# IBM/mcp-context-forge

Hardware: AMD Instinct MI355X
Metric: tool_call_req_per_s (higher is better)
Workload: dtype bf16

## Files before the change

### mcp_context_forge_amd/gpu/classifier.py

```python

from __future__ import annotations

import torch

from ..models.classifier import HashedTextClassifier
from ..ops import hip


class GpuClassifier:
    def __init__(self, model: HashedTextClassifier, device: str = "cuda"):
        self.dim = model.dim
        self.hidden = model.hidden
        self.classes = model.classes
        assert self.dim % 64 == 0 and self.hidden % 128 == 0, "MFMA tile constraints"
        with torch.no_grad():
            self.w1t = model.w1.t().contiguous().to(device=device, dtype=torch.bfloat16)
            self.b1 = model.b1.to(device=device, dtype=torch.float32).contiguous()
            self.w2t = model.w2.t().contiguous().to(device=device, dtype=torch.bfloat16)
            self.b2 = model.b2.to(device=device, dtype=torch.float32).contiguous()

    def forward(self, feats_bf16: torch.Tensor) -> torch.Tensor:
        h = hip.gemm_bt(feats_bf16, self.w1t, self.b1, act=hip.ACT_GELU, out_bf16=True)
        return hip.gemv_head(h, self.w2t, self.b2, act=hip.ACT_SIGMOID)

    def forward_into(self, feats_bf16: torch.Tensor, h_buf: torch.Tensor,
                     scores_buf: torch.Tensor) -> None:
        hip.gemm_bt(feats_bf16, self.w1t, self.b1, act=hip.ACT_GELU, out_bf16=True, out=h_buf)
        hip.gemv_head(h_buf, self.w2t, self.b2, act=hip.ACT_SIGMOID, out=scores_buf)
```

### mcp_context_forge_amd/gpu/pipeline.py

```python

from __future__ import annotations

import asyncio
import json
import time
from typing import Any, Dict, List, Optional, Tuple

import numpy as np
import torch

from ..ops import dfa, hip
from ..ops.entropy import TOL as ENTROPY_TOL
from ..protocol import jsonrpc
from ..plugins.builtin import _walk_strings
from ..plugins.framework import PluginMode
from .batch import pack_texts, pad_rows
from .classifier import GpuClassifier
from .semcache import GpuSemanticCache, tool_hash

_NORMALIZE_TRIGGERS = ["\\t", "\\n", "\\r", "\\f", "\\u", "  ", '" ', ' "',
                       "[" + chr(0x80) + "-" + chr(0xFF) + "]"]

_SCHEMA_NEST_PATTERNS = [":\\{", ":\\["]

_TYPED_PAT = {
    "string": '"{k}":"',
    "number": '"{k}":[0-9\\-]',
    "integer": '"{k}":[0-9\\-]',
    "boolean": '"{k}":[tf]',
    "array": '"{k}":\\[',
}


class _ToolMeta:
    __slots__ = ("tool", "name", "tid", "itype", "thash", "native_kind", "native_client",
                 "client", "handler", "schema_mode", "required_bits", "typed_pairs",
                 "has_output_schema", "original_name", "reachable", "host_chain", "a2a_fast")

    def __init__(self):
        self.schema_mode = "host"
        self.required_bits = 0
        self.typed_pairs: List[Tuple[int, int]] = []
        self.native_kind = -1
        self.native_client = None
        self.client = None
        self.handler = None
        self.has_output_schema = False
        self.host_chain = False
        self.a2a_fast = False


class _PackedRows:

    __slots__ = ("blob", "offs")

    def __init__(self, blob: bytes, offs: np.ndarray):
        self.blob = blob
        self.offs = offs

    def __len__(self) -> int:
        return max(int(self.offs.shape[0]) - 1, 0)

    def __getitem__(self, i: int) -> bytes:
        return self.blob[int(self.offs[i]):int(self.offs[i + 1])]


class _IndexedUsers:

    __slots__ = ("users", "uidx")

    def __init__(self, users: List[Optional[str]], uidx: np.ndarray):
# ... 126 lines not shown

        self.banks["postmeta"] = hip.DeviceScanTables(
            dfa.compile_literals(['"structuredContent"'], case_insensitive=False), device)

        self._bankset3 = hip.ScanBankSet(
            [(n, self.banks[n]) for n in ("pii", "regex", "harm", "postmeta", "secrets")
             if n in self.banks],
            device)
        self._bankset1: Optional[hip.ScanBankSet] = None
        self._graphs = None
        self._graphs3 = None

        self._slot_store = hip.store_new(self.semcache.capacity) if self.semcache is not None else 0
        self._exact_native = hip.cache_new(self.exact_cache.ttl) if self.exact_cache is not None else 0

        def _strtable(items):
            blob = b"".join(x.encode() for x in items)
            off = np.zeros(len(items) + 1, dtype=np.int32)
            for i, x in enumerate(items):
                off[i + 1] = off[i] + len(x.encode())
            return np.frombuffer(blob, dtype=np.uint8).copy() if blob else np.zeros(1, dtype=np.uint8), off

        from ..models.classifier import category_names

        self._deny_tab = _strtable(self.deny.words if self.deny else [])
        self._harm_tab = _strtable(self.harm.cats if self.harm else [])
        self._mod_tab = _strtable(category_names(self.moderation.model.classes) if self.moderation else [])

        self._meta_gen = -1
        self._plugins_ver = -1
        self._toolmap = 0
        self._meta_list: List[_ToolMeta] = []
        self._tool_meta: Dict[str, _ToolMeta] = {}
        self._schema_bank: Optional[hip.DeviceScanTables] = None
        self._schema_pat_ids: Dict[str, int] = {}
        self._nest_bits = 0

        self.batches = 0
        self.requests = 0
        self.fast_path = 0
        self.slow_path = 0
        self.blocked = 0
        self.cache_hits = 0
        self.post_rewrites = 0
        self.post_c = 0
        self.post_c_punt = 0
        self.py_fallback = 0
        self.host_bound = 0
        self.secrets_routed = 0
        import os as _os

        self.timing_enabled = bool(_os.environ.get("FORGE_PIPELINE_TIMING"))
        self.timing: Dict[str, float] = {}

    def _schema_pattern(self, pat: str) -> int:
        pid = self._schema_pat_ids.get(pat)
        if pid is None:
            pid = len(self._schema_pat_ids)
            self._schema_pat_ids[pat] = pid
        return pid

    def _esc_key(self, k: str) -> Optional[str]:
        if not k or not all(c.isalnum() or c == "_" for c in k):
            return None
        return k

    def _compile_tool_schema(self, meta: _ToolMeta, schema: Optional[dict]) -> None:
        if self.schema_guard is None or not schema:
            meta.schema_mode = "trivial"
            return
        if not (schema.get("properties") or schema.get("required") or
                schema.get("additionalProperties") is False or schema.get("anyOf") or
                schema.get("allOf") or schema.get("oneOf")):
            meta.schema_mode = "trivial"
            return
        props = schema.get("properties") or {}
        required = schema.get("required") or []
        if schema.get("additionalProperties") is False or schema.get("anyOf") or \
           schema.get("allOf") or schema.get("oneOf"):
            meta.schema_mode = "host"
            return
        req_bits = 0
        pairs: List[Tuple[int, int]] = []
        for k, sub in props.items():
            ek = self._esc_key(k)
            ty = sub.get("type") if isinstance(sub, dict) else None
            extra = isinstance(sub, dict) and any(
                c in sub for c in ("enum", "const", "pattern", "minimum", "maximum", "minLength",
                                   "maxLength", "minItems", "maxItems", "properties", "items",
                                   "anyOf", "allOf", "oneOf", "exclusiveMinimum", "exclusiveMaximum"))
            if ek is None or extra or (ty is not None and not isinstance(ty, str)) or \
               (ty is not None and ty not in _TYPED_PAT and ty not in ("object", "null")):
                meta.schema_mode = "host"
                return
            present = self._schema_pattern(f'"{ek}":')
            if ty in _TYPED_PAT:
                typed = self._schema_pattern(_TYPED_PAT[ty].format(k=ek))
                pairs.append((present, typed))
            if k in required:
                req_bits |= 1 << present
        for k in required:
            if k not in props:
                ek = self._esc_key(k)
                if ek is None:
                    meta.schema_mode = "host"
                    return
# ... 863 lines not shown
                    else:
                        punted.append(j)
                nat_set = set(nat_idx)
                py_js = [j for j in rewrite_js if j not in nat_set] + punted
                py_js.sort()
        self._toc("rw_c", t_sub)
        t_sub = self._tic()

        for j in py_js:
            mt = self._meta_list[tool_idx[j]]
            r = int(rows[j])
            idb = self._id_bytes(blob, env, r)
            try:
                args = json.loads(blob[args_b[j]:args_e[j]].tobytes() or b"{}")
            except Exception:
                responses[r] = self._splice_error(idb, jsonrpc.INVALID_PARAMS, "invalid arguments")
                continue
            if self.deny is not None and self._t_rw_deny[tool_idx[j]]:
                hay = _text_of(args)
                hay = hay.lower() if self.deny.case_insensitive else hay
                word = next((w for w in self.deny.words
                             if (w.lower() if self.deny.case_insensitive else w) in hay), None)
                if word is not None:
                    responses[r] = self._splice_error(
                        idb, jsonrpc.POLICY_DENIED, f"deny_filter: deny word {word!r} present")
                    self.blocked += 1
                    continue
            status, payload = self._apply_rewrites(
                mt.name, args,
                do_norm=bool(norm_m[j]) if norm_m is not None else True,
                do_regex=bool(regex_m[j]) if regex_m is not None else True,
                do_pii=bool(pii_m[j]) if pii_m is not None else True,
                pii_bits=int(pii_m[j]) if pii_m is not None else -1)
            if status == "__block__":
                responses[r] = self._splice_error(idb, jsonrpc.POLICY_DENIED, payload)
                self.blocked += 1
                continue
            if self.harm is not None and self._t_rw_harm[tool_idx[j]]:
                hay2 = _text_of(payload).lower()
                for w, ph in enumerate(self.harm.phrases):
                    if ph.lower() in hay2:
                        harm_c[j] = w
                        break
            ok_items.append((j, payload))
        self._toc("rw_pyloop", t_sub)
        if not ok_items:
            return None
        t_sub = self._tic()

        texts2 = [scan_bytes[j] if j in scan_bytes
                  else json.dumps(a, separators=(",", ":"), sort_keys=True, default=str).encode()
                  for (j, a) in ok_items]
        scores2_t = None
        if self.classifier is not None:
            data2, beg2, end2 = pack_texts(texts2, self.device)
            f2, _ = hip.featurize(data2, beg2, end2, self.feat_dim, pad_to=128)
            scores2_t = self.classifier.forward(f2)[: len(ok_items)]

        self._toc("rw_launch", t_sub)
        async def finish() -> List[Tuple[int, Any]]:
            return await self._finish_rewrite(ok_items, harm_c, schema_c, scores2_t,
                                              blob, env, rows, tool_idx, hit, hit_slot, responses)

        return finish

    async def _finish_rewrite(self, ok_items, harm_c, schema_c, scores2_t,
                              blob, env, rows, tool_idx, hit, hit_slot,
                              responses: List[Optional[bytes]]) -> List[Tuple[int, Any]]:
        t_sub = self._tic()
        if scores2_t is not None:
            await self._await_gpu()
        self._toc("rw_sync", t_sub)
        t_sub = self._tic()
        scores2 = scores2_t.cpu().numpy() if scores2_t is not None else None

        mod_on = scores2 is not None and self._enforcing(self.moderation)
        sc_max = scores2.max(axis=1) if mod_on else None
        sc_arg = scores2.argmax(axis=1) if mod_on else None
        mod_thr = self.moderation.threshold if mod_on else 0.0
        sg_on = self._enforcing(self.schema_guard)
        if mod_on:
            from ..models.classifier import category_names
            cat_names = category_names(scores2.shape[1])
        if sg_on:
            from ..utils.jsonschema import validate as _validate
        mod_app, harm_cats = self._t_mod_app, (self.harm.cats if self.harm else [])

        out: List[Tuple[int, Any]] = []
        for jj, (j, args2) in enumerate(ok_items):
            ti = tool_idx[j]
            if mod_on and mod_app[ti] and float(sc_max[jj]) >= mod_thr:
                r = int(rows[j])
                cat = cat_names[int(sc_arg[jj])]
                responses[r] = self._splice_error(
                    self._id_bytes(blob, env, r), jsonrpc.POLICY_DENIED,
                    f"content_moderation: moderation: category {cat} score {float(sc_max[jj]):.3f}")
                self.blocked += 1
                continue
            hj = harm_c.get(j, -1)
            if hj >= 0:
                r = int(rows[j])
                cat = harm_cats[hj] if hj < len(harm_cats) else "?"
                responses[r] = self._splice_error(
                    self._id_bytes(blob, env, r), jsonrpc.POLICY_DENIED,
                    f"harmful_content_detector: harmful content ({cat})")
                self.blocked += 1
                continue
            if sg_on and schema_c.get(j, 2) == 1:
                pass
            elif sg_on and self._meta_list[ti].schema_mode != "trivial":
                mt = self._meta_list[ti]
                if isinstance(args2, bytes):
                    args2 = json.loads(args2)
                errs = _validate(args2 or {}, mt.tool.get("input_schema") or {})
                if errs:
                    r = int(rows[j])
                    responses[r] = self._splice_error(
                        self._id_bytes(blob, env, r), jsonrpc.POLICY_DENIED,
                        "schema_guard: schema violation: " + "; ".join(errs[:5]))
                    self.blocked += 1
                    continue
            if hit[j]:
                r = int(rows[j])
                res = self._cache_result_bytes(int(hit_slot[j]))
                idb = self._id_bytes(blob, env, r)
                if idb is not None and res is not None:
                    responses[r] = self._splice_result(idb, res)
# ... 373 lines not shown

            new = _walk_strings(result, fn)
            if found and self.pii.action == "block" and self._enforcing(self.pii):
                return rb, True, f"pii_filter: PII detected: {sorted(set(found))}"
            if found and self.pii.action == "mask":
                result = new
        if mt.has_output_schema and isinstance(result, dict):
            from ..utils.jsonschema import validate as _validate

            payload = result.get("structuredContent", result)
            errs = _validate(payload, mt.tool.get("output_schema") or {})
            if errs:
                result = {"content": [{"type": "text", "text": "output schema violation: " + "; ".join(errs[:3])}],
                          "isError": True}
        if self.harm is not None and self._enforcing(self.harm) and self._applies(self.harm, name):
            hay = json.dumps(result, separators=(",", ":"), sort_keys=True, default=str).lower()
            for phrase, cat in zip(self.harm.phrases, self.harm.cats):
                if phrase.lower() in hay:
                    return rb, True, f"harmful_content_detector: harmful content ({cat})"
        if self.toon is not None and self._applies(self.toon, name) and isinstance(result, dict):
            new = self.toon.encode_result(result)
            if new is not None:
                result = new
        if self.out_guard is not None and isinstance(result, dict):
            total = sum(len(c.get("text", "")) for c in result.get("content", []) if isinstance(c, dict))
            if total > self.out_guard.max_chars and self.out_guard.action == "truncate":
                result = dict(result)
                result["content"] = [
                    {**c, "text": c["text"][: self.out_guard.max_chars]}
                    if isinstance(c, dict) and isinstance(c.get("text"), str) else c
                    for c in result.get("content", [])
                ]
        is_err = bool(isinstance(result, dict) and result.get("isError"))
        return json.dumps(result, separators=(",", ":"), default=str).encode(), is_err, None

    def _breaker_record(self, name: str, is_error: bool) -> None:
        b = self.breaker
        st = b._st(name)
        st["results"].append(is_error)
        if len(st["results"]) > b.window:
            st["results"] = st["results"][-b.window:]
        if len(st["results"]) >= b.window and (sum(st["results"]) / len(st["results"])) >= b.error_threshold:
            st["open_until"] = time.monotonic() + b.cooldown
            st["results"] = []

    def stats(self) -> Dict[str, Any]:
        out = {
            "timing_s": {k: round(v, 4) for k, v in self.timing.items()} if self.timing_enabled else None,
            "batches": self.batches, "requests": self.requests, "fast_path": self.fast_path,
            "slow_path": self.slow_path, "blocked": self.blocked, "cache_hits": self.cache_hits,
            "host_bound": self.host_bound, "secrets_routed": self.secrets_routed,
            "post_rewrites": self.post_rewrites, "post_c": self.post_c,
            "post_c_punt": self.post_c_punt, "py_fallback": self.py_fallback,
            "banks": {k: {"states": v.n_states, "classes": v.n_classes} for k, v in self.banks.items()},
        }
        if self.semcache is not None:
            out["semcache"] = self.semcache.stats()
        return out
```

### mcp_context_forge_amd/ops/build.py

```python

from __future__ import annotations

import os
import subprocess
import sys
from pathlib import Path

CSRC = Path(__file__).parent / "csrc"
LIB = Path(__file__).parent / "libforge_hip.so"
ARCH = os.environ.get("PYTORCH_ROCM_ARCH", "gfx950")
HIPCC = os.environ.get("HIPCC", "/opt/rocm/bin/hipcc")

SOURCES = ["scan.hip", "entropy.hip", "featurize.hip", "json_guard.hip", "gemm_bf16.hip", "runtime.hip",
           "gemm_v2.hip", "envelope.cpp", "upstream.cpp", "fastpath.cpp", "rewrite.cpp", "pool.cpp"]


PYBRIDGE = Path(__file__).parent / "forge_pybridge.so"
EDGE = Path(__file__).parent / "forge_edge.so"
HEY = Path(__file__).parent / "forge_hey"


def needs_build() -> bool:
    if not LIB.exists():
        return True
    lib_mtime = LIB.stat().st_mtime
    watched = [CSRC / f for f in SOURCES] + sorted(CSRC.glob("*.h"))
    return any(f.stat().st_mtime > lib_mtime for f in watched)


def build_pybridge(force: bool = False, verbose: bool = True) -> Path:
    src = CSRC / "pybridge.c"
    if not force and PYBRIDGE.exists() and PYBRIDGE.stat().st_mtime > src.stat().st_mtime:
        return PYBRIDGE
    import sysconfig

    cc = os.environ.get("CC", "gcc")
    cmd = [cc, "-O2", "-fPIC", "-shared", f"-I{sysconfig.get_paths()['include']}",
           "-o", str(PYBRIDGE), str(src)]
    if verbose:
        print("[forge-pybridge]", " ".join(cmd), file=sys.stderr)
    subprocess.run(cmd, check=True)
    return PYBRIDGE


def build_edge(force: bool = False, verbose: bool = True) -> Path:
    src = CSRC / "edge.cpp"
    newest = max(src.stat().st_mtime, (CSRC / "edge_pack.hpp").stat().st_mtime)
    if not force and EDGE.exists() and EDGE.stat().st_mtime > newest:
        return EDGE
    import sysconfig

    cxx = os.environ.get("CXX", "g++")
    cmd = [cxx, "-O2", "-std=c++17", "-fPIC", "-shared", "-pthread",
           f"-I{sysconfig.get_paths()['include']}", "-o", str(EDGE), str(src)]
    if verbose:
        print("[forge-edge]", " ".join(cmd), file=sys.stderr)
    subprocess.run(cmd, check=True)
    return EDGE


def build_hey(force: bool = False, verbose: bool = True) -> Path:
    src = CSRC / "forge_hey.cpp"
    if not force and HEY.exists() and HEY.stat().st_mtime > src.stat().st_mtime:
        return HEY
    cxx = os.environ.get("CXX", "g++")
    cmd = [cxx, "-O2", "-std=c++17", "-pthread", "-o", str(HEY), str(src)]
    if verbose:
# ... 31 lines not shown
```

### mcp_context_forge_amd/ops/csrc/forge_api.h

```cpp
#ifndef FORGE_API_H
#define FORGE_API_H

#include <stdint.h>

#define FORGE_ACT_NONE 0
#define FORGE_ACT_GELU 1
#define FORGE_ACT_SIGMOID 2

#define FORGE_ERR_SHAPE 9001
#define FORGE_ERR_ACT 9002
#define FORGE_ERR_GEMV_K 9003
#define FORGE_ERR_ROW_ALIGN 9004

#define FORGE_SCAN_LDS_LIMIT (64 * 1024)
#define FORGE_SCAN_TABLE_BYTES(n_states, n_classes) \
    ((int64_t)(n_states) * (n_classes) * 2 + 256 + (int64_t)(n_states) * 4)

typedef void (*forge_task_fn)(int index, void* ctx);

#ifdef __cplusplus
extern "C" {
#endif


// ... 74 lines not shown

int64_t forge_decide(
    const uint8_t* blob, const int32_t* id_beg, const int32_t* id_end,
    const int32_t* args_beg, const int32_t* args_end, const int32_t* tool_idx,
    const int32_t* name_beg, const int32_t* name_end,
    const uint32_t* deny_m, const uint32_t* harm_m, const uint32_t* pii_m,
    const uint32_t* regex_m, const uint32_t* norm_m, const uint32_t* schema_m,
    const uint8_t* mod_block, const int32_t* mod_cat, const float* mod_score,
    const uint8_t* hit, const int32_t* hit_slot, const uint64_t* user_hash, int m,
    const uint32_t* tool_flags, const uint32_t* tool_required_bits,
    const uint64_t* tool_typed_pairs,
    const int32_t* tname_beg, const int32_t* tname_end, const uint8_t* tname_blob,
    const int8_t* tool_native_kind, uint32_t nest_bits,
    const uint8_t* deny_words, const int32_t* deny_off, int n_deny,
    const uint8_t* harm_cats, const int32_t* harm_off, int n_harm,
    const uint8_t* mod_cats, const int32_t* mod_off, int n_mod,
    void* slot_store, void* exact_cache, double now,
    int32_t* state, int32_t* native_kind_out, int8_t* reason_out,
    uint8_t* arena, int64_t arena_cap, int64_t* resp_beg, int64_t* resp_end);

int64_t forge_finalize(
    const uint8_t* blob, const int32_t* id_beg, const int32_t* id_end,
    const int32_t* args_beg, const int32_t* args_end, const int32_t* tool_idx,
    const uint64_t* user_hash, int m, const int32_t* rows, int n_rows,
    const uint8_t* res_blob, const int64_t* res_beg, const int64_t* res_end,
    const uint8_t* needs_host,
    const int32_t* tname_beg, const int32_t* tname_end, const uint8_t* tname_blob,
    const uint32_t* tool_flags,
    void* exact_cache, double now, double exact_ttl,
    uint8_t* arena, int64_t arena_cap, int64_t* resp_beg, int64_t* resp_end,
    uint8_t* is_error_out, uint8_t* cacheable_out);

int64_t forge_rewrite_rows(
    const uint8_t* blob, const int32_t* args_beg, const int32_t* args_end, int n,
    const uint8_t* do_flags, const uint32_t* pii_want,
    uint32_t pii_active_mask, int pii_mode, int norm_collapse, int norm_strip,
    const uint8_t* deny_blob, const int32_t* deny_off, int n_deny, int deny_ci,
    int32_t* status, uint32_t* found_bits, int32_t* deny_hit,
    uint8_t* arena, int64_t arena_cap,
    int64_t* out_beg, int64_t* out_end, int64_t* scan_beg, int64_t* scan_end,
    const uint8_t* harm_blob, const int32_t* harm_off, int n_harm, int32_t* harm_out,
    const uint8_t* sk_blob, const int32_t* sk_beg, const int32_t* sk_end,
    const int8_t* sk_type, const uint8_t* sk_req,
    const int32_t* sk_lo, const int32_t* sk_hi, uint8_t* schema_out);

int64_t forge_post_rows(
    const uint8_t* blob, const int64_t* res_beg, const int64_t* res_end, int n,
    const uint8_t* do_flags, uint32_t pii_active_mask, int pii_mode,
    const uint8_t* harm_blob, const int32_t* harm_off, int n_harm,
    int64_t toon_min_size, double toon_min_savings,
    int32_t* status, uint32_t* found_bits, int32_t* harm_hit, uint8_t* is_err,
    uint8_t* arena, int64_t arena_cap, int64_t* out_beg, int64_t* out_end);

#ifdef __cplusplus
}
#endif

#endif
```

### mcp_context_forge_amd/ops/hip.py

```python

from __future__ import annotations

import ctypes
import os
from functools import lru_cache
from typing import List, Optional, Tuple

import numpy as np
import torch

from . import entropy
from .dfa import ScanTables


class ForgeHipError(RuntimeError):
    pass


_KINDS = {"p": ctypes.c_void_p, "s": ctypes.c_char_p, "i": ctypes.c_int, "u": ctypes.c_uint32,
          "l": ctypes.c_int64, "d": ctypes.c_double, "v": None}


def _sig(ret: str, args: str):
    return _KINDS[ret], [_KINDS[c] for c in args.replace(" ", "")]


_API = {
    "forge_scan": _sig("i", "ppp i ppp ii pp p"),
    "forge_scan_multi": _sig("i", "ppp i p ii p p"),
    "forge_token_entropy": _sig("i", "ppp i pi pppp p"),
    "forge_featurize": _sig("i", "ppp ii pp p"),
    "forge_json_guard": _sig("i", "ppp i ii pp p"),
    "forge_gemm_bt": _sig("i", "pppp iii ii p"),
    "forge_gemm_bt_v2": _sig("i", "pppp iii ii p"),
    "forge_gemv_head": _sig("i", "pppp iii i p"),
    "forge_rows_argmax_merge": _sig("i", "p iii p pp p"),
    "forge_rows_gather_scatter_bf16": _sig("i", "ppp p p ii p"),
    "forge_verify_dot": _sig("i", "ppp p ii p"),
    "forge_parallel_for": _sig("v", "i p p"),
    "forge_parse_envelopes": _sig("i", "pp i p pp pp pp"),
    "forge_upstream_call_batch": _sig("l", "ppp p i s p l pp"),
    "forge_store_new": _sig("p", "i"),
    "forge_store_put": _sig("v", "p i p l"),
    "forge_store_put_batch": _sig("v", "p p i p pp"),
    "forge_store_get": _sig("l", "p i p l"),
    "forge_store_free": _sig("v", "p"),
    "forge_cache_new": _sig("p", "d"),
    "forge_cache_free": _sig("v", "p"),
    "forge_toolmap_new": _sig("p", "ppp i"),
    "forge_toolmap_free": _sig("v", "p"),
    "forge_toolmap_resolve": _sig("v", "p p pp i p"),
    "forge_decide": _sig("l", "p pp pp p pp pppppp ppp pp p i ppp ppp p u ppi ppi ppi pp d ppp pl pp"),
    "forge_finalize": _sig("l", "p pp pp p p i pi ppp p ppp p p dd pl pp pp"),
    "forge_rewrite_rows": _sig("l", "ppp i pp u i ii pp ii ppp pl pp pp pp i p ppp pp pp p"),
    "forge_post_rows": _sig("l", "ppp i p u i pp i l d pppp pl pp"),
}


@lru_cache(maxsize=1)
def _load() -> ctypes.CDLL:
    from .build import LIB, build

    if not LIB.exists():
        build()
    lib = ctypes.CDLL(str(LIB))
    for name, (restype, argtypes) in _API.items():
        fn = getattr(lib, name)
        fn.restype = restype
        fn.argtypes = argtypes
    return lib


def available() -> bool:
    try:
        return torch.cuda.is_available() and _load() is not None
    except Exception:
        return False


def _stream() -> ctypes.c_void_p:
    return ctypes.c_void_p(torch.cuda.current_stream().cuda_stream)


def _check(name: str, rc: int) -> None:
    if rc != 0:
        raise ForgeHipError(f"{name} failed with code {rc}")


def _ptr(t: Optional[torch.Tensor]) -> ctypes.c_void_p:
    return ctypes.c_void_p(t.data_ptr()) if t is not None else ctypes.c_void_p(0)


def _np_ptr(a: Optional[np.ndarray]) -> ctypes.c_void_p:
    return ctypes.c_void_p(a.ctypes.data) if a is not None else ctypes.c_void_p(0)


def _call_growing(cap: int, fn):
    while True:
        arena = np.empty(cap, dtype=np.uint8)
        n = int(fn(arena, cap))
        if n >= 0:
            return arena, n
        cap = -n + 4096


class DeviceScanTables:

    def __init__(self, tables: ScanTables, device: str = "cuda"):
# ... 373 lines not shown
            _np_ptr(harm_blob), _np_ptr(harm_off), n_harm, _np_ptr(harm_hit),
            _np_ptr(sk_blob), _np_ptr(sk_beg), _np_ptr(sk_end),
            _np_ptr(sk_type), _np_ptr(sk_req),
            _np_ptr(sk_lo), _np_ptr(sk_hi), _np_ptr(schema_ok))

    arena, _ = _call_growing(int((args_end - args_beg).sum()) * 2 + n * 32 + 4096, call)
    return status, found, deny_hit, harm_hit, schema_ok, arena, out_beg, out_end, scan_beg, scan_end


def post_rows(res_blob: np.ndarray, res_beg: np.ndarray, res_end: np.ndarray,
              do_flags: np.ndarray, pii_active_mask: int, pii_mode: int,
              harm_blob: Optional[np.ndarray] = None,
              harm_off: Optional[np.ndarray] = None,
              toon_min_size: int = 1 << 60, toon_min_savings: float = 1.0):
    n = res_beg.shape[0]
    lib = _load()
    status = np.empty(n, dtype=np.int32)
    found = np.empty(n, dtype=np.uint32)
    harm_hit = np.empty(n, dtype=np.int32)
    is_err = np.empty(n, dtype=np.uint8)
    out_beg = np.empty(n, dtype=np.int64)
    out_end = np.empty(n, dtype=np.int64)
    n_harm = (harm_off.shape[0] - 1) if harm_off is not None else 0

    def call(arena, cap):
        return lib.forge_post_rows(
            _np_ptr(res_blob), _np_ptr(res_beg), _np_ptr(res_end), n,
            _np_ptr(do_flags),
            ctypes.c_uint32(pii_active_mask), pii_mode,
            _np_ptr(harm_blob), _np_ptr(harm_off), n_harm,
            ctypes.c_int64(toon_min_size), ctypes.c_double(toon_min_savings),
            _np_ptr(status), _np_ptr(found), _np_ptr(harm_hit), _np_ptr(is_err),
            _np_ptr(arena), cap, _np_ptr(out_beg), _np_ptr(out_end))

    arena, _ = _call_growing(int((res_end - res_beg).sum()) * 2 + n * 64 + 4096, call)
    return status, found, harm_hit, is_err, arena, out_beg, out_end


TF_REACHABLE, TF_DENY, TF_PII, TF_REGEX, TF_NORM, TF_MOD, TF_HARM = (1 << i for i in range(7))
TF_SCHEMA_FAST, TF_SCHEMA_HOST, TF_CACHE, TF_EXACT, TF_BREAKER_OPEN = (1 << i for i in range(7, 12))
ST_DISPATCH_NATIVE, ST_ANSWERED, ST_REWRITE, ST_HOST_SCHEMA, ST_DISPATCH_PY = 0, 1, 2, 3, 4


def store_get(store: int, slot: int) -> Optional[bytes]:
    lib = _load()
    buf = ctypes.create_string_buffer(4096)
    n = lib.forge_store_get(ctypes.c_void_p(store), slot, buf, 4096)
    if n < 0 or n == 0:
        return None
    if n > 4096:
        buf = ctypes.create_string_buffer(int(n))
        n = lib.forge_store_get(ctypes.c_void_p(store), slot, buf, int(n))
    return buf.raw[:int(n)]
```

Measured before the change: 321,300.

## Score small rewrite rescan batches with a native CPU classifier instead of GPU

Adds a multithreaded C++ implementation of the hashed-text classifier (featurize, GEMM with GELU, sigmoid head) that mirrors the GPU path's bf16 rounding. The rewrite path uses it when the rescan batch has at most 256 rows, which skips the host-to-device packing, kernel launches, GPU sync and device-to-host copy for small batches. Larger batches still take the GPU path. The trade-off is CPU time spent on the dense hidden-layer math and small numeric differences from the GPU kernels.

Measured after the change: 318,700. About the same (-0.8%).

```diff
diff --git a/loadtest/rescan_bench.py b/loadtest/rescan_bench.py
--- /dev/null
+++ b/loadtest/rescan_bench.py
@@ -0,0 +1,82 @@
+
+from __future__ import annotations
+
+import argparse
+import json
+import random
+import statistics
+import sys
+import time
+from pathlib import Path
+
+sys.path.insert(0, str(Path(__file__).resolve().parents[1]))
+
+import torch
+
+
+def make_texts(n: int, seed: int = 1):
+    rng = random.Random(seed)
+    out = []
+    for _ in range(n):
+        k = rng.randrange(3)
+        if k == 0:
+            a = {"time": "2026-01-%02dT%02d:%02d:%02dZ" % (rng.randrange(1, 29), rng.randrange(24),
+                                                         rng.randrange(60), rng.randrange(60)),
+                 "source_timezone": rng.choice(["UTC", "America/New_York", "Europe/London", "Asia/Tokyo"]),
+                 "target_timezone": rng.choice(["UTC", "America/Chicago", "Europe/Berlin", "Asia/Kolkata"])}
+        elif k == 1:
+            a = {"timezone": rng.choice(["UTC", "America/New_York", "Europe/Paris"])}
+        else:
+            a = {"msg": f"payload {rng.randrange(1 << 30)} lorem ipsum dolor sit amet", "n": rng.randrange(100)}
+        a["note"] = "contact me at [EMAIL_REDACTED]" if rng.random() < 0.5 else "this is spaced text"
+        out.append(json.dumps(a, separators=(",", ":"), sort_keys=True).encode())
+    return out
+
+
+def median_us(fn, iters: int, warmup: int = 10) -> float:
+    for _ in range(warmup):
+        fn()
+    times = []
+    for _ in range(iters):
+        t0 = time.perf_counter()
+        fn()
+        times.append(time.perf_counter() - t0)
+    return statistics.median(times) * 1e6
+
+
+def main() -> None:
+    ap = argparse.ArgumentParser()
+    ap.add_argument("--iters", type=int, default=50)
+    ap.add_argument("--sizes", default="4,16,64,256,1024")
+    a = ap.parse_args()
+
+    from mcp_context_forge_amd.gpu.batch import pack_texts
+    from mcp_context_forge_amd.gpu.classifier import GpuClassifier
+    from mcp_context_forge_amd.models.classifier import HashedTextClassifier
+    from mcp_context_forge_amd.ops import hip
+
+    model = HashedTextClassifier().eval()
+    gc = GpuClassifier(model)
+
+    def gpu_path(texts):
+        torch.cuda.synchronize()
+        data, beg, end = pack_texts(texts, "cuda")
+        f, _ = hip.featurize(data, beg, end, model.dim, pad_to=128)
+        s = gc.forward(f)[: len(texts)].cpu().numpy()
+        torch.cuda.synchronize()
+        return s
+
+    rows = []
+    for n in [int(x) for x in a.sizes.split(",")]:
+        texts = make_texts(n)
+        diff = float(abs(gc.score_rows(texts) - gpu_path(texts)).max())
+        rows.append({"n": n,
+                     "native_us": round(median_us(lambda: gc.score_rows(texts), a.iters), 1),
+                     "gpu_us": round(median_us(lambda: gpu_path(texts), a.iters), 1),
+                     "max_abs_diff": diff})
+    wins = [r["n"] for r in rows if r["native_us"] < r["gpu_us"]]
+    print(json.dumps({"iters": a.iters, "rows": rows, "native_wins_up_to": max(wins) if wins else 0}))
+
+
+if __name__ == "__main__":
+    main()
diff --git a/mcp_context_forge_amd/gpu/classifier.py b/mcp_context_forge_amd/gpu/classifier.py
--- a/mcp_context_forge_amd/gpu/classifier.py
+++ b/mcp_context_forge_amd/gpu/classifier.py
@@ -1,6 +1,9 @@
 
 from __future__ import annotations
 
+from typing import List
+
+import numpy as np
 import torch
 
 from ..models.classifier import HashedTextClassifier
@@ -8,6 +11,8 @@
 
 
 class GpuClassifier:
+    _host = 0
+
     def __init__(self, model: HashedTextClassifier, device: str = "cuda"):
         self.dim = model.dim
         self.hidden = model.hidden
@@ -18,6 +23,26 @@
             self.b1 = model.b1.to(device=device, dtype=torch.float32).contiguous()
             self.w2t = model.w2.t().contiguous().to(device=device, dtype=torch.bfloat16)
             self.b2 = model.b2.to(device=device, dtype=torch.float32).contiguous()
+            self._host = hip.modscore_new(
+                model.w1.detach().cpu().to(torch.bfloat16), model.b1.detach().cpu(),
+                model.w2.detach().cpu().t().contiguous().to(torch.bfloat16), model.b2.detach().cpu())
+        if not self._host:
+            raise hip.ForgeHipError(
+                f"forge_modscore_new refused dim={self.dim} hidden={self.hidden} classes={self.classes}")
+
+    def score_rows(self, texts: List[bytes]) -> np.ndarray:
+        return hip.modscore_rows(self._host, texts)
+
+    def close(self) -> None:
+        if self._host:
+            hip.modscore_free(self._host)
+            self._host = 0
+
+    def __del__(self):
+        try:
+            self.close()
+        except Exception:
+            pass
 
     def forward(self, feats_bf16: torch.Tensor) -> torch.Tensor:
         h = hip.gemm_bt(feats_bf16, self.w1t, self.b1, act=hip.ACT_GELU, out_bf16=True)
diff --git a/mcp_context_forge_amd/gpu/pipeline.py b/mcp_context_forge_amd/gpu/pipeline.py
--- a/mcp_context_forge_amd/gpu/pipeline.py
+++ b/mcp_context_forge_amd/gpu/pipeline.py
@@ -17,6 +17,8 @@
 from .batch import pack_texts, pad_rows
 from .classifier import GpuClassifier
 from .semcache import GpuSemanticCache, tool_hash
+
+RESCAN_NATIVE_MAX = 256
 
 _NORMALIZE_TRIGGERS = ["\\t", "\\n", "\\r", "\\f", "\\u", "  ", '" ', ' "',
                        "[" + chr(0x80) + "-" + chr(0xFF) + "]"]
@@ -249,6 +251,9 @@
 
         self.timing_enabled = bool(_os.environ.get("FORGE_PIPELINE_TIMING"))
         self.timing: Dict[str, float] = {}
+        self.rescan_native_max = int(_os.environ.get("FORGE_RESCAN_NATIVE_MAX", RESCAN_NATIVE_MAX))
+        self.rescan_native = 0
+        self.rescan_gpu = 0
 
     def _schema_pattern(self, pat: str) -> int:
         pid = self._schema_pat_ids.get(pat)
@@ -1218,12 +1223,16 @@
                   else json.dumps(a, separators=(",", ":"), sort_keys=True, default=str).encode()
                   for (j, a) in ok_items]
         scores2_t = None
-        if self.classifier is not None:
+        if self.classifier is not None and len(ok_items) <= self.rescan_native_max:
+            scores2_t = self.classifier.score_rows(texts2)
+            self.rescan_native += len(ok_items)
+            self._toc("rw_score", t_sub)
+        elif self.classifier is not None:
             data2, beg2, end2 = pack_texts(texts2, self.device)
             f2, _ = hip.featurize(data2, beg2, end2, self.feat_dim, pad_to=128)
             scores2_t = self.classifier.forward(f2)[: len(ok_items)]
-
-        self._toc("rw_launch", t_sub)
+            self.rescan_gpu += len(ok_items)
+            self._toc("rw_launch", t_sub)
         async def finish() -> List[Tuple[int, Any]]:
             return await self._finish_rewrite(ok_items, harm_c, schema_c, scores2_t,
                                               blob, env, rows, tool_idx, hit, hit_slot, responses)
@@ -1234,11 +1243,14 @@
                               blob, env, rows, tool_idx, hit, hit_slot,
                               responses: List[Optional[bytes]]) -> List[Tuple[int, Any]]:
         t_sub = self._tic()
-        if scores2_t is not None:
-            await self._await_gpu()
-        self._toc("rw_sync", t_sub)
-        t_sub = self._tic()
-        scores2 = scores2_t.cpu().numpy() if scores2_t is not None else None
+        if isinstance(scores2_t, np.ndarray):
+            scores2 = scores2_t
+        else:
+            if scores2_t is not None:
+                await self._await_gpu()
+            self._toc("rw_sync", t_sub)
+            t_sub = self._tic()
+            scores2 = scores2_t.cpu().numpy() if scores2_t is not None else None
 
         mod_on = scores2 is not None and self._enforcing(self.moderation)
         sc_max = scores2.max(axis=1) if mod_on else None
@@ -1718,6 +1730,7 @@
             "host_bound": self.host_bound, "secrets_routed": self.secrets_routed,
             "post_rewrites": self.post_rewrites, "post_c": self.post_c,
             "post_c_punt": self.post_c_punt, "py_fallback": self.py_fallback,
+            "rescan_native": self.rescan_native, "rescan_gpu": self.rescan_gpu,
             "banks": {k: {"states": v.n_states, "classes": v.n_classes} for k, v in self.banks.items()},
         }
         if self.semcache is not None:
diff --git a/mcp_context_forge_amd/ops/build.py b/mcp_context_forge_amd/ops/build.py
--- a/mcp_context_forge_amd/ops/build.py
+++ b/mcp_context_forge_amd/ops/build.py
@@ -12,7 +12,8 @@
 HIPCC = os.environ.get("HIPCC", "/opt/rocm/bin/hipcc")
 
 SOURCES = ["scan.hip", "entropy.hip", "featurize.hip", "json_guard.hip", "gemm_bf16.hip", "runtime.hip",
-           "gemm_v2.hip", "envelope.cpp", "upstream.cpp", "fastpath.cpp", "rewrite.cpp", "pool.cpp"]
+           "gemm_v2.hip", "envelope.cpp", "upstream.cpp", "fastpath.cpp", "rewrite.cpp", "pool.cpp",
+           "modscore.cpp"]
 
 
 PYBRIDGE = Path(__file__).parent / "forge_pybridge.so"
diff --git a/mcp_context_forge_amd/ops/csrc/forge_api.h b/mcp_context_forge_amd/ops/csrc/forge_api.h
--- a/mcp_context_forge_amd/ops/csrc/forge_api.h
+++ b/mcp_context_forge_amd/ops/csrc/forge_api.h
@@ -150,6 +150,15 @@
     int32_t* status, uint32_t* found_bits, int32_t* harm_hit, uint8_t* is_err,
     uint8_t* arena, int64_t arena_cap, int64_t* out_beg, int64_t* out_end);
 
+void* forge_modscore_new(const uint16_t* w1_dh_bf16, const float* b1,
+                         const uint16_t* w2t_bf16, const float* b2,
+                         int dim, int hidden, int classes);
+
+void forge_modscore_free(void* h);
+
+int forge_modscore_rows(void* h, const uint8_t* blob, const int64_t* beg, const int64_t* end,
+                        int n, float* out_scores);
+
 #ifdef __cplusplus
 }
 #endif
diff --git a/mcp_context_forge_amd/ops/csrc/modscore.cpp b/mcp_context_forge_amd/ops/csrc/modscore.cpp
--- /dev/null
+++ b/mcp_context_forge_amd/ops/csrc/modscore.cpp
@@ -0,0 +1,197 @@
+
+#include <math.h>
+#include <stdint.h>
+#include <string.h>
+
+#include <algorithm>
+#include <new>
+#include <vector>
+
+#include "forge_api.h"
+
+namespace {
+
+constexpr uint32_t FNV_OFFSET = 0x811C9DC5u;
+constexpr uint32_t FNV_PRIME = 0x01000193u;
+constexpr int MAX_DIM = 8192;
+constexpr int MAX_CLASSES = 32;
+constexpr int ROWS_PER_TASK = 4;
+constexpr int MAX_TASKS = 15;
+constexpr int LANES = 8;
+
+inline bool is_word(uint8_t b) {
+    return (b >= '0' && b <= '9') || (b >= 'A' && b <= 'Z') || (b >= 'a' && b <= 'z') || b == '_';
+}
+inline uint8_t lower(uint8_t b) { return (b >= 'A' && b <= 'Z') ? (uint8_t)(b + 0x20) : b; }
+
+inline float bf16_to_f(uint16_t v) {
+    uint32_t u = (uint32_t)v << 16;
+    float f;
+    memcpy(&f, &u, 4);
+    return f;
+}
+
+inline float bf16_rne(float f) {
+    uint32_t u;
+    memcpy(&u, &f, 4);
+    uint32_t lsb = (u >> 16) & 1;
+    u += 0x7fff + lsb;
+    u &= 0xffff0000u;
+    memcpy(&f, &u, 4);
+    return f;
+}
+
+inline float tanh_fast(float u) {
+    u = (u > -10.0f) ? u : -10.0f;
+    u = (u < 10.0f) ? u : 10.0f;
+    const float x = 2.0f * u;
+    const float fx = x * 1.44269504088896341f + 0.5f;
+    float fn = (float)(int)fx;
+    fn -= (fn > fx) ? 1.0f : 0.0f;
+    const float r = (x - fn * 0.693359375f) - fn * -2.12194440e-4f;
+    float p = 1.9875691500e-4f;
+    p = p * r + 1.3981999507e-3f;
+    p = p * r + 8.3334519073e-3f;
+    p = p * r + 4.1665795894e-2f;
+    p = p * r + 1.6666665459e-1f;
+    p = p * r + 5.0000001201e-1f;
+    const float y = (p * r) * r + r + 1.0f;
+    const uint32_t bits = (uint32_t)((int)fn + 127) << 23;
+    float scale;
+    memcpy(&scale, &bits, 4);
+    const float e = y * scale;
+    return 1.0f - 2.0f / (e + 1.0f);
+}
+
+inline float gelu_tanh(float x) {
+    const float c = 0.7978845608028654f;
+    float x3 = x * x * x;
+    return 0.5f * x * (1.0f + tanh_fast(c * (x + 0.044715f * x3)));
+}
+
+inline float sigmoidf_(float x) { return 1.0f / (1.0f + expf(-x)); }
+
+struct Model {
+    int dim, hidden, classes;
+    std::vector<float> w1;
+    std::vector<float> b1;
+    std::vector<float> w2t;
+    std::vector<float> b2;
+};
+
+struct Scratch {
+    std::vector<uint32_t> counts;
+    std::vector<int32_t> touched;
+    std::vector<float> pre;
+};
+
+Scratch& scratch_for(const Model& m) {
+    static thread_local Scratch s;
+    if ((int)s.counts.size() < m.dim) s.counts.resize(m.dim, 0u);
+    if ((int)s.touched.capacity() < m.dim) s.touched.reserve(m.dim);
+    if ((int)s.pre.size() < m.hidden) s.pre.resize(m.hidden);
+    return s;
+}
+
+void score_row(const Model& m, Scratch& s, const uint8_t* p, int64_t len, float* out) {
+    const uint32_t mask = (uint32_t)(m.dim - 1);
+    uint32_t* counts = s.counts.data();
+    s.touched.clear();
+    uint32_t h = FNV_OFFSET;
+    bool in_tok = false;
+    for (int64_t i = 0; i <= len; ++i) {
+        if (i < len && is_word(p[i])) {
+            h = (h ^ (uint32_t)lower(p[i])) * FNV_PRIME;
+            in_tok = true;
+            continue;
+        }
+        if (in_tok) {
+            uint32_t k = h & mask;
+            if (counts[k]++ == 0) s.touched.push_back((int32_t)k);
+        }
+        h = FNV_OFFSET;
+        in_tok = false;
+    }
+
+    uint64_t ss = 0;
+    for (int32_t k : s.touched) ss += (uint64_t)counts[k] * counts[k];
+    const float inv = ss ? 1.0f / sqrtf((float)ss) : 0.0f;
+
+    const int H = m.hidden;
+    float* __restrict__ pre = s.pre.data();
+    const float* __restrict__ b1 = m.b1.data();
+    for (int j = 0; j < H; ++j) pre[j] = b1[j];
+    for (int32_t k : s.touched) {
+        const float v = bf16_rne((float)counts[k] * inv);
+        counts[k] = 0;
+        const float* __restrict__ w = m.w1.data() + (size_t)k * H;
+        for (int j = 0; j < H; ++j) pre[j] += v * w[j];
+    }
+    for (int j = 0; j < H; ++j) pre[j] = bf16_rne(gelu_tanh(pre[j]));
+
+    const int Hv = H - H % LANES;
+    for (int c = 0; c < m.classes; ++c) {
+        const float* __restrict__ w = m.w2t.data() + (size_t)c * H;
+        float acc[LANES] = {0};
+        for (int j = 0; j < Hv; j += LANES)
+            for (int l = 0; l < LANES; ++l) acc[l] += pre[j + l] * w[j + l];
+        float tail = 0.0f;
+        for (int j = Hv; j < H; ++j) tail += pre[j] * w[j];
+        float sum = ((acc[0] + acc[4]) + (acc[2] + acc[6])) + ((acc[1] + acc[5]) + (acc[3] + acc[7]));
+        out[c] = sigmoidf_(m.b2[c] + (sum + tail));
+    }
+}
+
+struct RowsCtx {
+    const Model* m;
+    const uint8_t* blob;
+    const int64_t* beg;
+    const int64_t* end;
+    int n, tasks;
+    float* out;
+};
+
+void rows_task(int t, void* vctx) {
+    const RowsCtx& c = *static_cast<const RowsCtx*>(vctx);
+    const int lo = (int)((int64_t)c.n * t / c.tasks), hi = (int)((int64_t)c.n * (t + 1) / c.tasks);
+    Scratch& s = scratch_for(*c.m);
+    for (int r = lo; r < hi; ++r) {
+        int64_t len = c.end[r] - c.beg[r];
+        score_row(*c.m, s, c.blob + c.beg[r], len > 0 ? len : 0, c.out + (size_t)r * c.m->classes);
+    }
+}
+
+}
+
+extern "C" void* forge_modscore_new(const uint16_t* w1_dh_bf16, const float* b1,
+                                    const uint16_t* w2t_bf16, const float* b2,
+                                    int dim, int hidden, int classes) {
+    if (!w1_dh_bf16 || !b1 || !w2t_bf16 || !b2) return nullptr;
+    if (dim < 1 || dim > MAX_DIM || (dim & (dim - 1)) != 0) return nullptr;
+    if (hidden < 1 || classes < 1 || classes > MAX_CLASSES) return nullptr;
+    Model* m = new (std::nothrow) Model();
+    if (!m) return nullptr;
+    m->dim = dim;
+    m->hidden = hidden;
+    m->classes = classes;
+    m->w1.resize((size_t)dim * hidden);
+    for (size_t i = 0; i < m->w1.size(); ++i) m->w1[i] = bf16_to_f(w1_dh_bf16[i]);
+    m->w2t.resize((size_t)classes * hidden);
+    for (size_t i = 0; i < m->w2t.size(); ++i) m->w2t[i] = bf16_to_f(w2t_bf16[i]);
+    m->b1.assign(b1, b1 + hidden);
+    m->b2.assign(b2, b2 + classes);
+    return m;
+}
+
+extern "C" void forge_modscore_free(void* h) { delete static_cast<Model*>(h); }
+
+extern "C" int forge_modscore_rows(void* h, const uint8_t* blob, const int64_t* beg,
+                                   const int64_t* end, int n, float* out_scores) {
+    if (!h || n < 0) return FORGE_ERR_SHAPE;
+    if (n == 0) return 0;
+    if (!blob || !beg || !end || !out_scores) return FORGE_ERR_SHAPE;
+    RowsCtx c{static_cast<const Model*>(h), blob, beg, end, n, 1, out_scores};
+    c.tasks = std::max(1, std::min(n / ROWS_PER_TASK, MAX_TASKS));
+    forge_parallel_for(c.tasks, rows_task, &c);
+    return 0;
+}
diff --git a/mcp_context_forge_amd/ops/csrc/modscore_driver.cpp b/mcp_context_forge_amd/ops/csrc/modscore_driver.cpp
--- /dev/null
+++ b/mcp_context_forge_amd/ops/csrc/modscore_driver.cpp
@@ -0,0 +1,198 @@
+
+#include <math.h>
+#include <stdio.h>
+#include <stdlib.h>
+#include <string.h>
+
+#include <string>
+#include <thread>
+#include <vector>
+
+#include "forge_api.h"
+
+static int fails = 0;
+#define CHECK(cond)                                                        \
+    do {                                                                   \
+        if (!(cond)) {                                                     \
+            fprintf(stderr, "CHECK failed %s:%d: %s\n", __FILE__, __LINE__, #cond); \
+            fails++;                                                       \
+        }                                                                  \
+    } while (0)
+
+static uint32_t rng_state = 2463534242u;
+static uint32_t rnd() {
+    rng_state = rng_state * 1664525u + 1013904223u;
+    return rng_state >> 8;
+}
+
+static uint16_t to_bf16(float f) {
+    uint32_t u;
+    memcpy(&u, &f, 4);
+    u += 0x7fff + ((u >> 16) & 1);
+    return (uint16_t)(u >> 16);
+}
+static float from_bf16(uint16_t v) {
+    uint32_t u = (uint32_t)v << 16;
+    float f;
+    memcpy(&f, &u, 4);
+    return f;
+}
+static float rne(float f) { return from_bf16(to_bf16(f)); }
+
+struct Weights {
+    int D, H, C;
+    std::vector<uint16_t> w1, w2t;
+    std::vector<float> b1, b2;
+};
+
+static Weights make_weights(int D, int H, int C, float scale) {
+    Weights w{D, H, C, {}, {}, {}, {}};
+    w.w1.resize((size_t)D * H);
+    w.w2t.resize((size_t)C * H);
+    w.b1.resize(H);
+    w.b2.resize(C);
+    for (auto& x : w.w1) x = to_bf16(scale * ((float)(rnd() % 2001) - 1000.0f) / 1000.0f);
+    for (auto& x : w.w2t) x = to_bf16(((float)(rnd() % 2001) - 1000.0f) / 4000.0f);
+    for (auto& x : w.b1) x = ((float)(rnd() % 2001) - 1000.0f) / 2000.0f;
+    for (auto& x : w.b2) x = ((float)(rnd() % 2001) - 1000.0f) / 2000.0f;
+    return w;
+}
+
+static bool is_word(uint8_t b) {
+    return (b >= '0' && b <= '9') || (b >= 'A' && b <= 'Z') || (b >= 'a' && b <= 'z') || b == '_';
+}
+
+static void reference(const Weights& w, const uint8_t* p, int64_t len, float* out) {
+    std::vector<float> cnt(w.D, 0.0f);
+    uint32_t h = 0x811C9DC5u;
+    bool in_tok = false;
+    for (int64_t i = 0; i < len; ++i) {
+        uint8_t b = p[i];
+        if (is_word(b)) {
+            if (b >= 'A' && b <= 'Z') b += 0x20;
+            h = (h ^ b) * 0x01000193u;
+            in_tok = true;
+        } else {
+            if (in_tok) cnt[h & (uint32_t)(w.D - 1)] += 1.0f;
+            h = 0x811C9DC5u;
+            in_tok = false;
+        }
+    }
+    if (in_tok) cnt[h & (uint32_t)(w.D - 1)] += 1.0f;
+    double ss = 0;
+    for (float c : cnt) ss += (double)c * c;
+    float inv = ss > 0 ? 1.0f / sqrtf((float)ss) : 0.0f;
+    std::vector<float> hid(w.H);
+    for (int j = 0; j < w.H; ++j) {
+        double pre = w.b1[j];
+        for (int k = 0; k < w.D; ++k)
+            if (cnt[k] != 0.0f) pre += (double)rne(cnt[k] * inv) * from_bf16(w.w1[(size_t)k * w.H + j]);
+        float x = (float)pre;
+        hid[j] = rne(0.5f * x * (1.0f + tanhf(0.7978845608028654f * (x + 0.044715f * x * x * x))));
+    }
+    for (int c = 0; c < w.C; ++c) {
+        double s = w.b2[c];
+        for (int j = 0; j < w.H; ++j) s += (double)hid[j] * from_bf16(w.w2t[(size_t)c * w.H + j]);
+        out[c] = 1.0f / (1.0f + expf(-(float)s));
+    }
+}
+
+static std::string random_row(int i) {
+    static const char* words[] = {"payload", "lorem", "ipsum", "Dolor", "SIT", "amet", "note", "contact",
+                                  "me", "at", "UTC", "Asia", "Tokyo", "n", "x_1", "007", "__"};
+    static const char* seps[] = {" ", ",", "\":\"", "\\", "\xc3\xa9", "{\"", "\"}", "/", "\t", "  "};
+    switch (i % 16) {
+    case 0: return "";
+    case 1: return "a";
+    case 2: return std::string(300, 'Q');
+    case 3: return "Hello hello HELLO";
+    case 4: return "-";
+    case 5: return "caf\xc3\xa9 na\xefve \\n\\t";
+    default: break;
+    }
+    std::string s;
+    int n = 1 + rnd() % 90;
+    for (int t = 0; t < n; ++t) {
+        s += words[rnd() % 17];
+        if (rnd() % 3 == 0) s += std::to_string(rnd() % 1000);
+        s += seps[rnd() % 10];
+    }
+    if (rnd() % 2) s += "tail";
+    return s;
+}
+
+static void run_model(int D, int H, int C, float scale, int rows, float tol) {
+    Weights w = make_weights(D, H, C, scale);
+    void* h = forge_modscore_new(w.w1.data(), w.b1.data(), w.w2t.data(), w.b2.data(), D, H, C);
+    CHECK(h != nullptr);
+    if (!h) return;
+
+    std::vector<uint8_t> blob = {'j', 'u', 'n', 'k'};
+    std::vector<int64_t> beg(rows), end(rows);
+    for (int i = 0; i < rows; ++i) {
+        std::string r = random_row(i);
+        beg[i] = (int64_t)blob.size();
+        blob.insert(blob.end(), r.begin(), r.end());
+        end[i] = (int64_t)blob.size();
+    }
+    std::vector<uint8_t> tight(blob.begin(), blob.end());
+
+    std::vector<float> got((size_t)rows * C, -1.0f), ref(C);
+    CHECK(forge_modscore_rows(h, tight.data(), beg.data(), end.data(), rows, got.data()) == 0);
+    float worst = 0;
+    for (int i = 0; i < rows; ++i) {
+        reference(w, tight.data() + beg[i], end[i] - beg[i], ref.data());
+        for (int c = 0; c < C; ++c) {
+            float d = fabsf(got[(size_t)i * C + c] - ref[c]);
+            if (d > worst) worst = d;
+        }
+    }
+    printf("D=%d H=%d C=%d rows=%d max|got-ref|=%.3g\n", D, H, C, rows, worst);
+    CHECK(worst <= tol);
+
+    std::vector<float> one(C);
+    for (int i = 0; i < rows; ++i) {
+        CHECK(forge_modscore_rows(h, tight.data(), beg.data() + i, end.data() + i, 1, one.data()) == 0);
+        CHECK(memcmp(one.data(), got.data() + (size_t)i * C, sizeof(float) * C) == 0);
+    }
+
+    std::vector<std::thread> th;
+    std::vector<std::vector<float>> outs(4, std::vector<float>((size_t)rows * C));
+    for (int t = 0; t < 4; ++t)
+        th.emplace_back([&, t] {
+            if (forge_modscore_rows(h, tight.data(), beg.data(), end.data(), rows, outs[t].data()) != 0)
+                outs[t][0] = -2.0f;
+        });
+    for (auto& t : th) t.join();
+    for (int t = 0; t < 4; ++t) CHECK(outs[t] == got);
+
+    CHECK(forge_modscore_rows(h, tight.data(), beg.data(), end.data(), 0, got.data()) == 0);
+    forge_modscore_free(h);
+}
+
+int main(int argc, char** argv) {
+    int rows = argc > 1 ? atoi(argv[1]) : 400;
+    int rounds = argc > 2 ? atoi(argv[2]) : 3;
+
+    Weights w = make_weights(64, 8, 3, 1.0f);
+    CHECK(forge_modscore_new(w.w1.data(), w.b1.data(), w.w2t.data(), w.b2.data(), 48, 8, 3) == nullptr);
+    CHECK(forge_modscore_new(w.w1.data(), w.b1.data(), w.w2t.data(), w.b2.data(), 64, 8, 0) == nullptr);
+    CHECK(forge_modscore_new(w.w1.data(), w.b1.data(), w.w2t.data(), w.b2.data(), 64, 8, 33) == nullptr);
+    CHECK(forge_modscore_new(w.w1.data(), w.b1.data(), w.w2t.data(), w.b2.data(), 64, 0, 3) == nullptr);
+    int64_t z = 0;
+    float o[3];
+    CHECK(forge_modscore_rows(nullptr, (const uint8_t*)"x", &z, &z, 1, o) == FORGE_ERR_SHAPE);
+    forge_modscore_free(nullptr);
+
+    for (int r = 0; r < rounds; ++r) {
+        run_model(4096, 256, 8, 1.0f / 64, rows, 2e-6f);
+        run_model(64, 131, 3, 0.5f, rows, 2e-4f);
+        run_model(8, 5, 32, 8.0f, rows / 4 + 1, 5e-3f);
+    }
+    if (fails) {
+        fprintf(stderr, "modscore driver: %d failure(s)\n", fails);
+        return 1;
+    }
+    printf("modscore driver ok\n");
+    return 0;
+}
diff --git a/mcp_context_forge_amd/ops/hip.py b/mcp_context_forge_amd/ops/hip.py
--- a/mcp_context_forge_amd/ops/hip.py
+++ b/mcp_context_forge_amd/ops/hip.py
@@ -54,6 +54,9 @@
     "forge_finalize": _sig("l", "p pp pp p p i pi ppp p ppp p p dd pl pp pp"),
     "forge_rewrite_rows": _sig("l", "ppp i pp u i ii pp ii ppp pl pp pp pp i p ppp pp pp p"),
     "forge_post_rows": _sig("l", "ppp i p u i pp i l d pppp pl pp"),
+    "forge_modscore_new": _sig("p", "pppp iii"),
+    "forge_modscore_free": _sig("v", "p"),
+    "forge_modscore_rows": _sig("i", "p ppp i p"),
 }
 
 
@@ -533,3 +536,49 @@
         buf = ctypes.create_string_buffer(int(n))
         n = lib.forge_store_get(ctypes.c_void_p(store), slot, buf, int(n))
     return buf.raw[:int(n)]
+
+
+
+def modscore_new(w1_bf16: torch.Tensor, b1: torch.Tensor, w2t_bf16: torch.Tensor,
+                 b2: torch.Tensor) -> int:
+    dim, hidden = w1_bf16.shape
+    classes = w2t_bf16.shape[0]
+    assert w1_bf16.dtype == torch.bfloat16 and w2t_bf16.dtype == torch.bfloat16
+    assert w2t_bf16.shape[1] == hidden and b1.numel() == hidden and b2.numel() == classes
+    w1 = w1_bf16.contiguous().view(torch.int16)
+    w2t = w2t_bf16.contiguous().view(torch.int16)
+    b1 = b1.to(torch.float32).contiguous()
+    b2 = b2.to(torch.float32).contiguous()
+    handle = _load().forge_modscore_new(_ptr(w1), _ptr(b1), _ptr(w2t), _ptr(b2),
+                                        dim, hidden, classes) or 0
+    if handle:
+        _modscore_classes[handle] = classes
+    return handle
+
+
+_modscore_classes: dict = {}
+
+
+def modscore_free(handle: int) -> None:
+    if _modscore_classes.pop(handle, None) is not None:
+        _load().forge_modscore_free(ctypes.c_void_p(handle))
+
+
+def modscore_rows(handle: int, texts, beg: Optional[np.ndarray] = None,
+                  end: Optional[np.ndarray] = None) -> np.ndarray:
+    classes = _modscore_classes[handle]
+    if beg is None:
+        n = len(texts)
+        offs = np.zeros(n + 1, dtype=np.int64)
+        np.cumsum(np.fromiter(map(len, texts), dtype=np.int64, count=n), out=offs[1:])
+        blob, beg, end = b"".join(texts), offs[:-1], offs[1:]
+    else:
+        n = beg.shape[0]
+        assert beg.dtype == np.int64 and end.dtype == np.int64 and end.shape[0] == n
+        beg, end = np.ascontiguousarray(beg), np.ascontiguousarray(end)
+        blob = texts
+    out = np.empty((n, classes), dtype=np.float32)
+    bp = blob if isinstance(blob, bytes) else _np_ptr(blob)
+    _check("forge_modscore_rows", _load().forge_modscore_rows(
+        ctypes.c_void_p(handle), bp, _np_ptr(beg), _np_ptr(end), n, _np_ptr(out)))
+    return out
```
